# forgi86/pyMPC

Hardware: AMD Instinct MI355X
Metric: QP-solves/sec (MPC steps/sec) at nx=12 nu=4 Np=30; max |u*-u*_ref| (higher is better)
Workload: dtype f64

## Files before the change

include/mpcqp.h:

```cpp
#ifndef MPCQP_H
#define MPCQP_H

#include <stdint.h>

#ifdef __cplusplus
extern "C" {
#endif

typedef struct mpcqp_handle mpcqp_handle;

enum mpcqp_error {
    MPCQP_OK = 0,
    MPCQP_ERR_ARG = -1,
    MPCQP_ERR_HIP = -2,
    MPCQP_ERR_NO_DEVICE = -3,
    MPCQP_ERR_UNSUPPORTED = -4,
    MPCQP_ERR_STATE = -5
};

enum mpcqp_status {
    MPCQP_SOLVED = 1, MPCQP_SOLVED_INACCURATE = 2, MPCQP_MAX_ITER_REACHED = -2,
    MPCQP_PRIMAL_INFEASIBLE = -3, MPCQP_PRIMAL_INFEASIBLE_INACCURATE = 3,
    MPCQP_DUAL_INFEASIBLE = -4, MPCQP_DUAL_INFEASIBLE_INACCURATE = 4,
    MPCQP_NON_CVX = -7, MPCQP_UNSOLVED = -10
// ... 16 lines not shown
    MPCQP_BACKEND_SWEEPS = 1,
    MPCQP_BACKEND_DENSE = 2,
    MPCQP_BACKEND_BCR = 3,
    MPCQP_BACKEND_BCR8 = 4,
    MPCQP_BACKEND_BCRT = 5
};
enum mpcqp_tuning {
    MPCQP_TUNE_NO_BALANCE = 1,
    MPCQP_TUNE_NO_LSTAGE = 2,
    MPCQP_TUNE_NO_GROUPING = 4,
    MPCQP_TUNE_NO_W8 = 8,
    MPCQP_TUNE_NO_QUEUE = 16,
    MPCQP_TUNE_NO_PARTS = 32,
    MPCQP_TUNE_QUEUE_SOLVES = 64,
    MPCQP_TUNE_EVEN_PARTS = 128,
    MPCQP_TUNE_ONE_LAUNCH_SOLVES = 1 << 29,
    MPCQP_TUNE_NO_SHARE = 1 << 30,
    MPCQP_TUNE_SLOTS_SHIFT = 24,
    MPCQP_TUNE_PACE_SHIFT = 8
};

typedef struct {
    int32_t status;
    int32_t iter;
    int32_t rho_updates;
    int32_t reserved;
    double obj_val;
    double pri_res, dua_res;
    double rho;
} mpcqp_info;
// ... 109 lines not shown
```

pympc_amd/_lib.py:

```python
import ctypes as C
import os

_HERE = os.path.dirname(os.path.abspath(__file__))
LIB_PATH = os.path.join(_HERE, 'libmpcqp_hip.so')

SYMBOLS = [
    'mpcqp_default_settings', 'mpcqp_status_string', 'mpcqp_last_error', 'mpcqp_device_count',
    'mpcqp_create', 'mpcqp_destroy', 'mpcqp_set_stream', 'mpcqp_synchronize',
    'mpcqp_setup', 'mpcqp_setup_qp', 'mpcqp_create_csc', 'mpcqp_setup_csc', 'mpcqp_update', 'mpcqp_update_vectors', 'mpcqp_warm_start', 'mpcqp_update_settings', 'mpcqp_solve',
    'mpcqp_mpc_step', 'mpcqp_step_host', 'mpcqp_mpc_run', 'mpcqp_mpc_loop', 'mpcqp_get_solution', 'mpcqp_get_u0', 'mpcqp_get_shape', 'mpcqp_get_dims', 'mpcqp_get_stream_bytes', 'mpcqp_get_work', 'mpcqp_get_occupancy', 'mpcqp_kernel_name', 'mpcqp_get_stats', 'mpcqp_get_launch_times', 'mpcqp_profile',
    'mpcqp_export_qp', 'mpcqp_get_scaling', 'mpcqp_debug_kkt_solve', 'mpcqp_get_iterate', 'mpcqp_iterate', 'mpcqp_refactor', 'mpcqp_share_factor', 'mpcqp_eq_solve',
]


class Settings(C.Structure):
    _fields_ = [('rho', C.c_double), ('sigma', C.c_double), ('alpha', C.c_double),
                ('eps_abs', C.c_double), ('eps_rel', C.c_double),
                ('eps_prim_inf', C.c_double), ('eps_dual_inf', C.c_double),
                ('adaptive_rho_tolerance', C.c_double),
                ('max_iter', C.c_int32), ('check_termination', C.c_int32), ('scaling', C.c_int32),
                ('adaptive_rho', C.c_int32), ('adaptive_rho_interval', C.c_int32), ('warm_start', C.c_int32),
                ('soft_constraints', C.c_int32), ('backend', C.c_int32), ('tuning', C.c_int32)]


BACKEND_AUTO, BACKEND_SWEEPS, BACKEND_DENSE, BACKEND_BCR, BACKEND_BCR8, BACKEND_BCRT = 0, 1, 2, 3, 4, 5
TUNE_NO_BALANCE, TUNE_NO_LSTAGE, TUNE_NO_GROUPING, TUNE_NO_W8, TUNE_NO_QUEUE, TUNE_NO_PARTS = 1, 2, 4, 8, 16, 32
TUNE_NO_SHARE = 1 << 30
TUNE_PACE_SHIFT = 8


class Info(C.Structure):
    _fields_ = [('status', C.c_int32), ('iter', C.c_int32), ('rho_updates', C.c_int32), ('reserved', C.c_int32),
                ('obj_val', C.c_double), ('pri_res', C.c_double), ('dua_res', C.c_double), ('rho', C.c_double)]


_pd = C.POINTER(C.c_double)


class Model(C.Structure):
    _fields_ = [(k, _pd) for k in ('Ad', 'Bd', 'Qx', 'QxN', 'Qu', 'QDu', 'xmin', 'xmax', 'umin', 'umax',
                                   'Dumin', 'Dumax', 'uref', 'eps_feas')]

# ... 82 lines not shown
```

pympc_amd/csrc/mpcqp.hip:

```cpp

#include <hip/hip_runtime.h>
#include <math.h>
#include <stdint.h>
#include <stdio.h>
#include <string.h>
#include <sched.h>
#include <algorithm>
#include <cstdio>
#include <cstdlib>
#include <string>
#include <vector>

#include "../../include/mpcqp.h"

#include "mpcqp_defs.h"

static inline void cpu_relax() {
#if defined(__x86_64__) || defined(__i386__)
    __builtin_ia32_pause();
#elif defined(__aarch64__)
    __asm__ __volatile__("yield");
#else
    __asm__ __volatile__("" ::: "memory");
#endif
// ... 42 lines not shown
    int device, batch;
    Lay L;
    Ptrs P;
    mpcqp_settings S;
    hipStream_t stream;
    bool own_stream, is_setup, lds_state;
    size_t smem_setup, smem_solve;
    std::vector<void *> allocs;
    double *u0_dev;
    int *pending_dev, *npending_dev;
    int *perm_dev;
    int *qperm_dev; bool qperm_set;
    int *vcur_dev, *vdone_dev; unsigned *vqueue_dev;
    std::vector<double> work_ema;
    int ncu, solves_since_balance, auto_balance;
    void *run_buf; size_t run_bytes;
    bool profiling;
    hipEvent_t ev0[MAXEV], ev1[MAXEV];
    long long ev_count;
    double run_ms;
    long long run_launches;
    int nevents;
    bool warm_x_pending;
    double *pin_in, *pin_out; void *pin_in_dev, *pin_out_dev;
    unsigned *done_dev; unsigned long long host_seq; int pin_stride; bool pin_tried;
    PackArgs pack;
    CscSeam *csc;
    double *vec_buf;
    bool step_blank;
    int *fown_dev; unsigned *nshared_dev;
// ... 71 lines not shown
    HIPCHK(hipMalloc(&q, count * sizeof(T) + 16));
    HIPCHK(hipMemsetAsync(q, 0, count * sizeof(T) + 16, h->stream));
    h->allocs.push_back(q);
    *p = (T *)q;
    return 0;
}

extern "C" int mpcqp_create(mpcqp_handle **out, int device, int batch, int nx, int nu, int Np, int Nc, const mpcqp_settings *s) {
    if (!out || batch < 1 || nx < 1 || nu < 1 || Np < 2 || Nc < 1 || Nc > Np) return fail(MPCQP_ERR_ARG, "mpcqp_create: bad dimensions");
    if (nx + nu > 128) return fail(MPCQP_ERR_UNSUPPORTED, "mpcqp_create: nx+nu > 128 is not implemented");
    int ndev = 0;
    if (hipGetDeviceCount(&ndev) != hipSuccess || ndev == 0) return fail(MPCQP_ERR_NO_DEVICE, "no HIP device available");
    if (device < 0 || device >= ndev) return fail(MPCQP_ERR_ARG, "mpcqp_create: bad device index");
    HIPCHK(hipSetDevice(device));
    mpcqp_handle *h = new mpcqp_handle();
    h->device = device; h->batch = batch; h->is_setup = false; h->u0_dev = nullptr; h->run_buf = nullptr; h->run_bytes = 0; h->perm_dev = nullptr; h->vcur_dev = nullptr; h->vdone_dev = nullptr; h->vqueue_dev = nullptr; h->qperm_dev = nullptr; h->qperm_set = false; h->solves_since_balance = 0; h->auto_balance = 1; h->ncu = 0;
    h->profiling = false; h->run_ms = 0.0; h->run_launches = 0; h->ev_count = 0; h->nevents = 0; h->stream = nullptr; h->own_stream = false;
    h->warm_x_pending = false;
    h->csc = nullptr; h->vec_buf = nullptr; h->step_blank = false;
    h->pin_in = h->pin_out = nullptr; h->pin_in_dev = h->pin_out_dev = nullptr; h->done_dev = nullptr; h->host_seq = 0; h->pin_stride = 0; h->pin_tried = false;
    if (s) h->S = *s; else mpcqp_default_settings(&h->S);
    h->L = make_layout(nx, nu, Np, Nc, h->S.soft_constraints);
    auto hip_fail = [&](hipError_t e, const char *what) { std::string msg = std::string(what) + ": " + hipGetErrorString(e); mpcqp_destroy(h); return fail(MPCQP_ERR_HIP, msg); };
    { hipError_t e = hipStreamCreate(&h->stream); if (e != hipSuccess) { h->stream = nullptr; return hip_fail(e, "hipStreamCreate"); } }
    h->own_stream = true;
    for (int i = 0; i < MAXEV; ++i) {
        hipError_t e = hipEventCreate(&h->ev0[i]); if (e != hipSuccess) return hip_fail(e, "hipEventCreate");
        e = hipEventCreate(&h->ev1[i]); if (e != hipSuccess) { hipEventDestroy(h->ev0[i]); return hip_fail(e, "hipEventCreate"); }
        h->nevents = i + 1;
    }
    const Lay &L = h->L;
// ... 35 lines not shown
                  : (long long)L.fhead + (long long)L.N * L.fstage;
    int rc = 0;
    rc |= dalloc(h, &P.model, B * L.model_sz); rc |= dalloc(h, &P.step, B * L.step_sz);
    rc |= dalloc(h, &P.D, B * L.n); rc |= dalloc(h, &P.E, B * L.m); rc |= dalloc(h, &P.c, B);
    rc |= dalloc(h, &P.omega, B * L.m); rc |= dalloc(h, &P.s, B * L.n); rc |= dalloc(h, &P.rho, B);
    rc |= dalloc(h, &P.F, (B + 1) * (size_t)P.fsz);
    rc |= dalloc(h, &h->fown_dev, B); rc |= dalloc(h, &h->nshared_dev, 4);
    rc |= dalloc(h, &P.x, B * L.n); rc |= dalloc(h, &P.z, B * L.m); rc |= dalloc(h, &P.y, B * L.m);
    rc |= dalloc(h, &P.xo, B * L.n); rc |= dalloc(h, &P.yo, B * L.m);
    rc |= dalloc(h, &P.dx, B * L.n); rc |= dalloc(h, &P.dy, B * L.m);
    rc |= dalloc(h, &P.qv, B * (size_t)(L.n_x + L.n_u));
    if (bcr) rc |= dalloc(h, &P.bws, B * (size_t)NS * BcrFmt::WSTAGE);
    if (L.NB == 128) rc |= dalloc(h, &P.bws, B * (size_t)HugeFmt::GWS);
    if (L.border) { rc |= dalloc(h, &P.Bb, B * (size_t)L.nu * L.N * L.NB); rc |= dalloc(h, &P.Zb, B * (size_t)L.nu * L.N * L.NB); rc |= dalloc(h, &P.Sig, B * (size_t)L.nu * L.nu); }
    rc |= dalloc(h, &P.Dt, B * L.n); rc |= dalloc(h, &P.Et, B * L.m);
    rc |= dalloc(h, &P.ctype, B * L.m); rc |= dalloc(h, &P.info, B); rc |= dalloc(h, &P.stats, 8);
        rc |= dalloc(h, &h->u0_dev, B * L.nu);
    rc |= dalloc(h, &P.work, B); rc |= dalloc(h, &h->perm_dev, B);
    rc |= dalloc(h, &h->vcur_dev, (size_t)std::max(4 * h->ncu, 1)); rc |= dalloc(h, &h->vqueue_dev, 4); rc |= dalloc(h, &h->vdone_dev, B); rc |= dalloc(h, &h->qperm_dev, B);
    rc |= dalloc(h, &P.tstamp, (size_t)TS_STRIDE * B);
    rc |= dalloc(h, &h->pending_dev, B); rc |= dalloc(h, &h->npending_dev, 4);
    if (h->S.tuning & MPCQP_TUNE_NO_BALANCE) h->auto_balance = 0;
    if (rc) { std::string msg = g_err; mpcqp_destroy(h); return fail(MPCQP_ERR_HIP, msg); }
    const int toplds = bcrt ? LATW_TOP_LDS(NS) + 2 : 0;
    const int fws = dense ? L.NR * L.dld + 2 * DenseFmt::ROWS + L.m + L.n : bcr ? BcrFmt::lds_doubles(h->L.nw, L.m + L.n, bcrt ? BcrFmt::top_count(NS) : 0) : (L.NB == 16 ? FactorCfg<16>::WS : L.NB == 32 ? FactorCfg<32>::WS : L.NB == 64 ? WideFmt::WS : HugeFmt::WS);
    const int need = std::max(fws, (L.border && !dense) ? 2 * L.nu * L.nu : 0);
    const int avail = L.tsz + (h->lds_state ? (int)state_doubles : 0) + toplds;
    if (avail < need) h->L.tsz += need - avail;
    h->smem_setup = sizeof(double) * ((size_t)smem_common_doubles(h->L) + (h->lds_state ? state_doubles : 0) + (size_t)toplds);
    {
        const size_t stage_doubles = 2 * (size_t)L.n + 3 * (size_t)L.m + (size_t)(L.n_x + L.n_u) + (L.border ? 2 * (size_t)L.nu * L.N * L.NB + (size_t)L.nu * L.nu : 0);
// ... 307 lines not shown
    const int full = h->ncu * occ;
    const int q = (h->S.tuning >> MPCQP_TUNE_SLOTS_SHIFT) & 0x1F;
    if (q) return std::max(1, std::min(full, h->ncu * q / 8));
    if (L.NB == 32 && occ == 2 && !h->lds_state && !L.lstage && nsteps >= 8 && 2 * h->batch <= 3 * full && 4 * h->batch > 3 * full && !(h->S.tuning & MPCQP_TUNE_NO_QUEUE)) return 3 * full / 4;
    return full;
}
static RunKArgs run_kernel_args(mpcqp_handle *h, const RunArgs &R0, int *grid) {
    RunKArgs A; A.L = h->L; A.P = h->P; A.S = h->S; A.R = R0;
    *grid = h->batch;
    const int slots = run_grid(h, R0.nsteps);
    if (h->ncu > 0 && h->batch > slots && h->vcur_dev && !R0.pin_in && !R0.pub && (R0.nsteps > 0 || (h->S.tuning & (MPCQP_TUNE_QUEUE_SOLVES | MPCQP_TUNE_ONE_LAUNCH_SOLVES))) && !(h->S.tuning & MPCQP_TUNE_NO_QUEUE)) {
        A.R.vcur = h->vcur_dev; A.R.vperm = ((R0.nsteps > 0 || (R0.part == 0 && (h->S.tuning & MPCQP_TUNE_ONE_LAUNCH_SOLVES))) && h->qperm_set) ? h->qperm_dev : h->P.perm;       A.R.vqueue = h->vqueue_dev;
        A.P.perm = h->vcur_dev;
        *grid = slots;
        if (R0.nsteps > 1 && !(h->S.tuning & MPCQP_TUNE_NO_PARTS)) {
            const int per_slot = ((h->S.tuning >> 16) & 0xFF) ? ((h->S.tuning >> 16) & 0xFF) : QUEUE_ITEMS_PER_SLOT;
            const int parts = std::min(R0.nsteps, (per_slot * slots + h->batch - 1) / h->batch);
            if (parts > 1) {
                const int np = std::min(parts, 16);
                int off = 0;
                for (int p = 0; p < np; ++p) {
                    A.R.voff[p] = off;
                    const int left = R0.nsteps - off, pl = np - p;
                    int len = pl == 1 ? left : std::max(1, std::min(left - (pl - 1), (2 * left + pl) / (pl + 1)));
                    if (h->S.tuning & MPCQP_TUNE_EVEN_PARTS) len = pl == 1 ? left : (left + pl - 1) / pl;
                    off += len;
                }
                A.R.voff[np] = R0.nsteps; A.R.vparts = np; A.R.vdone = h->vdone_dev;
            }
        }
    }
    return A;
}
template <int NB, bool LDSS, int NXT, int NUT, int MODE>
static int launch_run_t(mpcqp_handle *h, const RunArgs &R) {
    int grid;
    const RunKArgs A = run_kernel_args(h, R, &grid);
    if (A.R.vdone && hipMemsetAsync(h->vdone_dev, 0, sizeof(int) * (size_t)h->batch, h->stream) != hipSuccess) return MPCQP_ERR_HIP;
    if (R.nsteps > 0) {
        if (set_smem(k_mpc_run<NB, LDSS, NXT, NUT, MODE, true>, h->smem_solve)) return MPCQP_ERR_HIP;
        hipLaunchKernelGGL((k_mpc_run<NB, LDSS, NXT, NUT, MODE, true>), dim3(grid), dim3(NT), h->smem_solve, h->stream, A);
    } else {
        if (set_smem(k_mpc_run<NB, LDSS, NXT, NUT, MODE, false>, h->smem_solve)) return MPCQP_ERR_HIP;
        hipLaunchKernelGGL((k_mpc_run<NB, LDSS, NXT, NUT, MODE, false>), dim3(grid), dim3(NT), h->smem_solve, h->stream, A);
    }
    return 0;
// ... 381 lines not shown
    for (unsigned long long spins = 0; *flag != h->host_seq; ++spins) {
        if (spins < 20000) cpu_relax(); else sched_yield();
        if ((spins & 0xfffff) == 0xfffff) {
            hipError_t e = hipStreamQuery(h->stream);
            if (e != hipSuccess && e != hipErrorNotReady) return fail(MPCQP_ERR_HIP, std::string("mpcqp_step_host: ") + hipGetErrorString(e));
            if (e == hipSuccess && *flag != h->host_seq) { HIPCHK(hipStreamSynchronize(h->stream)); break; }
        }
    }
    __atomic_thread_fence(__ATOMIC_ACQUIRE);
    if (x) memcpy(x, h->pin_out, sizeof(double) * B * L.n);
    if (y) memcpy(y, h->pin_out + B * L.n, sizeof(double) * B * L.m);
    if (info) memcpy(info, h->pin_out + B * (L.n + L.m), sizeof(mpcqp_info) * B);
    return MPCQP_OK;
}

extern "C" int mpcqp_get_stats(mpcqp_handle *h, uint64_t *out4, int reset) {
    if (!h || !out4) return fail(MPCQP_ERR_ARG, "null argument");
    HIPCHK(hipSetDevice(h->device));
    HIPCHK(hipMemcpyAsync(out4, h->P.stats, 4 * sizeof(uint64_t), hipMemcpyDefault, h->stream));
#ifdef MPCQP_RUN_TIMING
    { uint64_t t[4]; hipMemcpy(t, h->P.stats + 4, sizeof(t), hipMemcpyDeviceToHost); fprintf(stderr, "phase wall-clock ticks: begin %llu admm %llu check %llu\n", (unsigned long long)t[0], (unsigned long long)t[1], (unsigned long long)t[2]);
      unsigned long long g[16]; hipMemcpyFromSymbol(g, HIP_SYMBOL(g_ticks), sizeof(g)); unsigned long long z[16] = {0}; hipMemcpyToSymbol(HIP_SYMBOL(g_ticks), z, sizeof(z));
      if (h->L.nw == 8) mpcqp_w8_ticks(g);
      { double tot = 0; for (int i = 0; i < 7; ++i) tot += (double)g[i]; if (tot <= 0) tot = 1;
        fprintf(stderr, "iteration cycles (thread 0, summed over workgroups): rhs %.1f%% fwd %.1f%% middle %.1f%% bwd %.1f%% t4 %.1f%% t5 %.1f%% t6 %.1f%% total %.3g;  outside the iterations (same unit): t7 %.3g t8 %.3g t9 %.3g;  check: setup+tail %.3g rows %.3g vars %.3g reduce %.3g decide %.3g\n",
                100 * g[0] / tot, 100 * g[1] / tot, 100 * g[2] / tot, 100 * g[3] / tot, 100 * g[4] / tot, 100 * g[5] / tot, 100 * g[6] / tot, tot, (double)g[7], (double)g[8], (double)g[9], (double)g[10], (double)g[11], (double)g[12], (double)g[13], (double)g[14]); } }
#endif
    if (reset) HIPCHK(hipMemsetAsync(h->P.stats, 0, 8 * sizeof(uint64_t), h->stream));
    HIPCHK(hipStreamSynchronize(h->stream));
    return MPCQP_OK;
}

extern "C" int mpcqp_get_launch_times(mpcqp_handle *h, uint64_t *out, int nsteps) {
    if (!h || !out || nsteps < 0 || nsteps > TS_STEPS) return fail(MPCQP_ERR_ARG, "mpcqp_get_launch_times: bad argument (0 <= nsteps <= 64)");
    HIPCHK(hipSetDevice(h->device));
    HIPCHK(hipMemcpy2DAsync(out, sizeof(uint64_t) * (size_t)(2 + nsteps), h->P.tstamp, sizeof(uint64_t) * (size_t)TS_STRIDE, sizeof(uint64_t) * (size_t)(2 + nsteps),
                            (size_t)h->batch, hipMemcpyDefault, h->stream));
    HIPCHK(hipStreamSynchronize(h->stream));
    return MPCQP_OK;
}

extern "C" int mpcqp_profile(mpcqp_handle *h, int enable, double *run_ms, int64_t *run_launches, int reset) {
    if (!h) return fail(MPCQP_ERR_ARG, "null handle");
// ... 187 lines not shown
```

pympc_amd/csrc/mpcqp_kernels.h:

```cpp
#pragma once


struct RunSmem { Smem S; double *X, *Z, *Y; };
template <bool LDSSTATE>
__device__ __forceinline__ RunSmem run_smem(const Lay &L, const Ptrs &P) {
    extern __shared__ __attribute__((aligned(16))) double sh[];
    RunSmem r; double *p = sh; smem_common(L, P, p, r.S);
    r.X = r.Z = r.Y = nullptr;
    if (LDSSTATE) { r.X = carve(p, L.n); r.Z = carve(p, L.m); r.Y = carve(p, L.m); }
    return r;
}

template <int OCC>
__device__ __noinline__ void run_group_factor_phase(int *frame_pin) {
    PHASE_PIN_USE(frame_pin);
    const RunKArgs &A = run_kargs();
    const Lay &L = A.L; const Ptrs &P = A.P;
    RunSmem r = run_smem<false>(L, P);
    const int b = inst_of(P.perm);
    factor_unshare(P, b);
    Ctx c{L, r.S.hot, P.model + (size_t)b * L.model_sz + L.hot_sz};
    factor_grouped(c, P.omega + (size_t)b * L.m, P.s + (size_t)b * L.n, P.c[b], P.F + (size_t)b * P.fsz, r.S.T, r.S.iflag, border_ptrs(L, P, r.S));
}

// ... 59 lines not shown
__device__ __forceinline__ void run_instance(const int k0, const int k1) {
    constexpr int OCC = run_occupancy(NB, MODE);
    const RunKArgs &A = run_kargs();
    const Lay &L = A.L; const Ptrs &P = A.P; const RunArgs &R = A.R;
    RunSmem rs = run_smem<LDSSTATE>(L, P);
    Smem &S = rs.S;
    const int b = inst_of(P.perm), tid = threadIdx.x;
    double *step = P.step + (size_t)b * L.step_sz;
    if (LOOP && tid == 0 && k0 == 0) P.tstamp[(size_t)TS_STRIDE * b] = wall_clock64();
    if (LOOP && tid == 0 && k0 == 0 && R.nsteps < TS_STEPS) {
        unsigned hw, xcc;
        asm volatile("s_getreg_b32 %0, hwreg(HW_REG_HW_ID)" : "=s"(hw));
        asm volatile("s_getreg_b32 %0, hwreg(HW_REG_XCC_ID)" : "=s"(xcc));
        P.tstamp[(size_t)TS_STRIDE * b + 2 + TS_STEPS - 1] = ((unsigned long long)(xcc & 15) << 32) | hw;
    }
    if (MODE >= MODE_BCRT && tid == 0) S.iflag[2] = 0;
    const double *step_src = step;
    if (!LOOP && R.inl_n) {
        for (int i = tid; i < R.inl_n; i += NT) step[i] = R.inl[i];
        step_src = R.inl;
    } else if (!LOOP && R.pin_in) {
        const double *src = R.pin_in + (size_t)b * R.pin_stride;
        if (R.pin_mask & 1) for (int i = tid; i < L.nx; i += NT) step[i] = src[i];
        if (R.pin_mask & 2) for (int i = tid; i < L.nu; i += NT) step[L.nx + i] = src[L.nx + i];
        if (R.pin_mask & 4) for (int i = tid; i < R.pin_xref; i += NT) step[L.nx + L.nu + i] = src[L.nx + L.nu + i];
        __syncthreads();
    }
    load_common(L, P.model + (size_t)b * L.model_sz, step_src, S);
    if (!LOOP && R.part == 3) {
        __syncthreads();
        { FramePin pin; run_factor_phase<NB, OCC>(&pin.v); }
        return;
    }
    const int nx = L.nx, nu = L.nu;
    for (int k = k0; k < k1; ++k) {
        if (LOOP) {
            double *un = S.T, *xn = S.T + 128, *xt = S.T + 256, *ym = S.T + 384, *inn = S.T + 512, *xu = S.T + 640;
            const size_t kb = (size_t)k * R.batch + b;
            const int ny = R.ny;
            const int status = k > k0 ? S.iflag[4] : P.info[b].status;
            if (tid < nu) un[tid] = status == MPCQP_SOLVED ? (k > k0 ? S.uo[tid] : P.xo[(size_t)b * L.n + L.ou + tid]) : S.hot[L.ouref + tid];
            if (tid < nx) xt[tid] = ny ? R.x_true[(size_t)b * nx + tid] : S.x0s[tid];
            __syncthreads();
            if (ny && tid < ny) {
                const double *C = R.C + (size_t)b * ny * nx + (size_t)tid * nx;
                double y = R.v ? R.v[kb * ny + tid] : 0.0, yh = 0.0;
                for (int j = 0; j < nx; ++j) { y += C[j] * xt[j]; yh += C[j] * S.x0s[j]; }
                ym[tid] = y; inn[tid] = y - yh;
                if (R.y_traj) R.y_traj[kb * ny + tid] = y;
            }
            if (tid < nx) {
// ... 19 lines not shown
                __syncthreads();
                if (tid < nx) {
                    const double *Ad = S.hot + L.oAd, *Bd = S.hot + L.oBd;
                    double acc = 0.0;
                    for (int j = 0; j < nx; ++j) acc += Ad[tid * nx + j] * xu[j];
                    for (int j = 0; j < nu; ++j) acc += Bd[tid * nu + j] * un[j];
                    xn[tid] = acc;
                }
                __syncthreads();
            }
            if (tid < nx) { S.x0s[tid] = xn[tid]; step[tid] = xn[tid]; }
            if (tid < nu) { S.um1s[tid] = un[tid]; step[nx + tid] = un[tid]; S.du0[tid] = S.hot[L.oDumin + tid] + un[tid]; S.du0[nu + tid] = S.hot[L.oDumax + tid] + un[tid]; }
            if (R.xref_traj) for (int i = tid; i < R.xref_blk; i += NT) { const double xr = R.xref_traj[kb * R.xref_blk + i]; step[nx + nu + i] = xr; if (i < nx) S.xrs[i] = xr; }
            __syncthreads();
        }
#ifdef MPCQP_RUN_TIMING
#define PHASE_CLOCK(i) { unsigned long long t_ = wall_clock64(); if (tid == 0) atomicAdd(&P.stats[4 + (i)], t_ - tphase); tphase = t_; }
        unsigned long long tphase = wall_clock64();
#else
#define PHASE_CLOCK(i)
#endif
        int iter = 0, term = 0;
        if (!LOOP && R.part == 2) {
            const mpcqp_info pi = P.info[b];
            iter = pi.iter;
            if (tid == 0) { S.iflag[1] = pi.rho_updates; S.iflag[3] = pi.reserved; }
        }
        else { FramePin pin; run_begin_phase<NB, LDSSTATE, OCC>(R.plain, (R.warm_x && k == 0) ? 1 : 0, &pin.v); }
        __syncthreads();
        PHASE_CLOCK(0)
        while (!term) {
            const int nxt = next_stop(iter, R.max_iter, R.chk, R.rho_every);
            term = __builtin_amdgcn_readfirstlane(run_admm<NB, LDSSTATE, NXT, NUT, MODE, OCC>(nxt - iter, R.plain ? -1 : iter));
            iter = nxt;
            __syncthreads();
            if constexpr (MODE >= MODE_BCRT) { if (!R.plain) iter = S.iflag[5]; }
            PHASE_CLOCK(1)
            if (term) break;
            { FramePin pin; term = run_check_phase<NB, LDSSTATE, OCC>(iter, stop_mode(iter, R.max_iter, R.chk, R.rho_every, R.plain != 0), &pin.v); }
            __syncthreads();
            PHASE_CLOCK(2)
            if (!LOOP && R.part == 1 && !term) {
                if (tid == 0) R.pending[atomicAdd(R.npending, 1)] = b;
                break;
            }
        }
        if (LOOP && tid == 0) {
            R.status_traj[(size_t)k * R.batch + b] = S.iflag[4];
            R.iter_traj[(size_t)k * R.batch + b] = iter;
            if (k < TS_STEPS) P.tstamp[(size_t)TS_STRIDE * b + 2 + k] = wall_clock64();
        }
        __syncthreads();
    }
    if (!LOOP && R.pub) {
        double *px = R.pub + (size_t)b * L.n, *py = R.pub + (size_t)R.batch * L.n + (size_t)b * L.m;
        for (int j = tid; j < L.n; j += NT) px[j] = P.xo[(size_t)b * L.n + j];
        for (int r = tid; r < L.m; r += NT) py[r] = P.yo[(size_t)b * L.m + r];
        mpcqp_info *pi = (mpcqp_info *)(R.pub + (size_t)R.batch * (L.n + L.m));
        if (tid == 0) pi[b] = P.info[b];
        __threadfence_system();
// ... 28 lines not shown
    const int nvirt = (!LOOP && R.part == 2) ? *R.npending : R.batch;
    const int nparts = (LOOP && R.vparts > 1) ? R.vparts : 1;
    for (;;) {
        if (threadIdx.x == 0) {
            const int v = (int)atomicAdd(R.vqueue, 1u);
            int entry = -1, ka = 0, kb = nrun;
            if (v < nvirt * nparts) {
                const int part = v / nvirt, idx = v - part * nvirt;
                entry = R.vperm ? R.vperm[idx] : idx;
                if (nparts > 1) { ka = R.voff[part]; kb = R.voff[part + 1]; }
                if (part > 0) {
                    volatile int *done = R.vdone + (entry & PERM_INST_MASK);
                    while (*done < ka) __builtin_amdgcn_s_sleep(16);
                }
                R.vcur[blockIdx.x] = entry;
            }
            s_item[0] = entry; s_item[1] = ka; s_item[2] = kb;
        }
        __syncthreads();
        const int entry = s_item[0], ka = s_item[1], kb = s_item[2];
        if (entry < 0) {
            if (threadIdx.x == 0 && atomicAdd(R.vqueue + 1, 1u) == gridDim.x - 1) { R.vqueue[1] = 0; __threadfence(); R.vqueue[0] = 0; }
            break;
        }
        __builtin_amdgcn_s_dcache_inv();
        __builtin_amdgcn_fence(__ATOMIC_ACQUIRE, "agent");
        run_instance<NB, LDSSTATE, NXT, NUT, MODE, LOOP>(ka, kb);
        __syncthreads();
        if (nparts > 1 && threadIdx.x == 0) { __threadfence(); *(volatile int *)(R.vdone + (entry & PERM_INST_MASK)) = kb; }
    }
}

template <int NB>
__global__ __launch_bounds__(NT) void k_export(Lay L, Ptrs P, double *Pd, double *Ad_, double *q, double *l, double *u) {
    extern __shared__ __attribute__((aligned(16))) double sh[];
    double *p = sh; Smem S; smem_common(L, P, p, S);
    const int b = inst_of(P.perm), tid = threadIdx.x;
    const double *model = P.model + (size_t)b * L.model_sz, *step = P.step + (size_t)b * L.step_sz;
    load_common(L, model, step, S);
    Ctx c{L, S.hot, model + L.hot_sz};
    if (!L.raw) build_q(c, step, S.Qv);
    __syncthreads();
// ... 132 lines not shown
```

pympc_amd/csrc/mpcqp_latw.h:

```cpp
#pragma once

constexpr int latw_owner(int , int , int kind, int t) { return kind == 1 ? NWAVES - 1 - t % NWAVES : t % NWAVES; }
#ifndef LATW_FUSE0
#define LATW_FUSE0 2
#endif
constexpr bool latw_fused(int N) { return LATW_FUSE0 && (N + 3) / 4 == NWAVES; }
constexpr bool latw_fused_back(int N) { return LATW_FUSE0 >= 2 && latw_fused(N); }
constexpr int LATW_F0 = 6;
constexpr int LATW_FB = 6;
constexpr int latw_slot(int N, int W, int Lq, int kq, int tq) {
    int s = latw_fused(N) ? LATW_F0 : 0;
    for (int pass = 0; pass < 2; ++pass)
        for (int li = 0; li < 2; ++li) {
            const int L = pass == 0 ? li : 1 - li;
            for (int kind = (pass == 0 ? 0 : 2); kind < (pass == 0 ? 2 : 3); ++kind)
                for (int t = 0; t < lat_count(N, L, kind); ++t) {
                    if (latw_fused(N) && L == 0 && kind < 2) continue;
                    if (latw_fused_back(N) && kind == 2) continue;
                    if (L == Lq && kind == kq && t == tq) return s;
                    if (latw_owner(N, L, kind, t) == W) s += lat_nfr(N, L, kind, t);
                }
        }
    return s;
}
// ... 308 lines not shown
    if constexpr (latw_fused_back(N)) {
        LATW_DISPATCH(wv, (latw_bwd_own<N, W>(fr, v)))
        TICK(4)
    } else {
        LATW_DISPATCH(wv, (latw_bwd1<N, W>(fr, v)))
        __syncthreads();
        TICK(4)
        LATW_DISPATCH(wv, (latw_bwd<N, W, 0, false>(fr, v)))
    }
}

enum { LATW_CONTINUE = 0, LATW_SOLVED = 1, LATW_GENERIC = 2 };
template <int NXT, int NUT, int NST>
__device__ int latw_check(double pv, double pv2, double ncq, double zA, double ysA, double omA, double zB, double ysB, double omB, double z0, double ys0, double om0,
                          double loA, double hiA, double loB, double hiB, double cc, int iter, int *frame_pin);

template <int NXT, int NUT, int NST>
__device__ __forceinline__ int admm_latw(const Lay &L, const HotPtrs &P, Smem &S, double *Xl, double *Zl, double *Yl, double alpha, int iters, int iter0) {
    constexpr int NB = 16, N = NST, NG = (N + 3) / 4, QN = (NG + NWAVES - 1) / NWAVES;
#ifdef MPCQP_RUN_TIMING
    const unsigned long long tf0_ = clock64();
#endif
#ifndef LATW_FAST
#define LATW_FAST 1
#endif
    const bool fast = LATW_FAST && iter0 >= 0 && L.hot_lds > L.hot_sz;
    static_assert(NXT + NUT <= NB, "16 x 16 stages");
    const int nx = NXT ? NXT : L.nx, nu = NUT ? NUT : L.nu, NR = L.N;
    const int b = inst_of(P.perm), tid = threadIdx.x, lane = tid & 63, wv = __builtin_amdgcn_readfirstlane(tid >> 6);
    gdouble *gx = (gdouble *)(P.x + (size_t)b * L.n), *gz = (gdouble *)(P.z + (size_t)b * L.m), *gy = (gdouble *)(P.y + (size_t)b * L.m);
// ... 151 lines not shown
        }
        __syncthreads();
        TICK(6)
    }
    iter += iters;
    if (!fast) break;
    TICK_START
    if constexpr (QN != 1) break;
    else {
        const RunArgs &R = run_kargs().R;
        if (stop_mode(iter, R.max_iter, R.chk, R.rho_every, R.plain != 0) != COLD_CHECK) break;
        int verdict;
        { FramePin pin; verdict = latw_check<NXT, NUT, NST>(pv[0], pv2[0], ncq[0], rA[0].z, rA[0].ys, rA[0].om, rB[0].z, rB[0].ys, rB[0].om, r0.z, r0.ys, r0.om,
                                                               loA[0], hiA[0], loB[0], hiB[0], cc, iter, &pin.v); }
        verdict = __builtin_amdgcn_readfirstlane(verdict);
        if (verdict == LATW_SOLVED) { term = 1; break; }
        if (verdict != LATW_CONTINUE) break;
        iters = next_stop(iter, R.max_iter, R.chk, R.rho_every) - iter;
        auto rt = [&](LatRow &r) { r.ys = cc * (r.ys * (r.om * cinv)) / r.om; r.w = r.om * (r.z - r.ys); };
        rt(rA[0]); rt(rB[0]);
        if (u0v) rt(r0);
        WA[sl[0]] = ok[0] ? rA[0].w : 0.0; WB[sl[0]] = ok[0] ? rB[0].w : 0.0;
        __syncthreads();
    }
    TICK(9)
    }
    TICK_START
    if (!term) {
        auto put_row = [&](const LatRow &r, int idx) { const double y = r.ys * (r.om * cinv); gz[idx] = r.z; gy[idx] = y; Zl[idx] = r.z; Yl[idx] = y; };
#pragma unroll
        for (int q = 0; q < QN; ++q) {
            if (ok[q]) {
// ... 16 lines not shown
```

pympc_amd/csrc/mpcqp_latw_check.h:

```cpp
#pragma once

template <int NXT, int NUT, int NST>
__device__ __noinline__ int latw_check(double pv, double pv2, double ncq, double zA, double ysA, double omA, double zB, double ysB, double omB, double z0, double ys0, double om0,
                                       double loA, double hiA, double loB, double hiB, double cc, int iter, int *frame_pin) {
    PHASE_PIN_USE(frame_pin);
    constexpr int NB = 16, N = NST, NG = (N + 3) / 4, VS = LAT_VS(N), NTOP = BcrFmt::top_count(N);
    static_assert(NG <= NWAVES, "one group of four stages per wave");
    const RunKArgs &KA = run_kargs();
    const Lay &L = KA.L; const Ptrs &PP = KA.P; const RunArgs &R = KA.R;
    RunSmem rs = run_smem<true>(L, PP);
    Smem &S = rs.S;
    const int nx = NXT ? NXT : L.nx, nu = NUT ? NUT : L.nu, NR = L.N;
    const int b = inst_of(PP.perm), tid = threadIdx.x, lane = tid & 63, wv = __builtin_amdgcn_readfirstlane(tid >> 6);
    const double cinv = 1.0 / cc;
    const double *hot = S.hot;
    double *Tc = S.T + NB, *Cc = Tc + VS;
    const double *TopL = rs.Y + L.m + ((smem_common_doubles(L) + L.n + 2 * L.m) & 1);
    const int a = 4 * ((lane >> 2) & 3) + (lane >> 4), J = lane & 3;
    const bool is_x = a < nx;
    const int jj = a - nx;
    const int s = wv < NG ? 4 * wv + J : 4 * NG, sl = s * NB + a;
    const bool ok = is_x ? s < NR : (a < nx + nu && s < NR - 1);
    const int e = s * nx + a, cu = s * nu + jj;
    const int pidx = is_x ? e : L.ou + cu, aidx = is_x ? e : L.ri + cu, bidx = is_x ? L.rs + e : L.rdu + nu + cu;
// ... 83 lines not shown
            S.iflag[4] = MPCQP_SOLVED;
            atomicAdd(&PP.stats[0], (unsigned long long)iter); atomicAdd(&PP.stats[1], (unsigned long long)inf.reserved);
            atomicAdd(&PP.stats[2], (unsigned long long)inf.rho_updates); atomicAdd(&PP.stats[3], 1ULL);
            PP.work[b] += (unsigned)iter;
            inf.reserved = 0;
            PP.info[b] = inf;
        }
        return LATW_SOLVED;
    }
    if (R.nsteps == 0 && R.part == 1) return LATW_GENERIC;
    if (!pc && nrm[7] > epi && vsum[1] < -epi * nrm[7]) return LATW_GENERIC;
    if (!dc && nrm[8] > edi && vsum[2] < -edi * nrm[8]) return LATW_GENERIC;
    if (tid == 0) S.iflag[3] += 1;
    return LATW_CONTINUE;
}
```

pympc_amd/csrc/mpcqp_qp.h:

```cpp
#pragma once

__device__ __forceinline__ double input_weight(double iu, double qu, double dk, double qdu) {
    double a = iu * qu, b = dk * qdu;
    asm volatile("" : "+v"(a), "+v"(b));
    return a + b;
}


template <class F>
__device__ __forceinline__ void A_row(const Ctx &c, int r, F f) {
    const Lay &L = c.L;
    if (r < L.rs) {
        int k = idiv(r, L.rnx), i = r - k * L.nx;
        f(-1.0, r);
        if (k > 0) {
            const double *a = c.Ad() + i * L.nx;
            int base = (k - 1) * L.nx;
            for (int j = 0; j < L.nx; ++j) f(a[j], base + j);
            int ku = min(k - 1, L.Nc - 1);
            const double *b = c.Bd() + i * L.nu;
            base = L.ou + ku * L.nu;
            for (int j = 0; j < L.nu; ++j) f(b[j], base + j);
        }
    } else if (r < L.ri) {
// ... 76 lines not shown
    } else if (r < L.ri) {
        int j = r - L.rs; int k = idiv(j, L.rnx); int i = j - k * L.nx;
        lo = c.hot[L.oxmin + i]; hi = c.hot[L.oxmax + i];
    } else if (r < L.rdu) {
        int cc = r - L.ri; int k = idiv(cc, L.rnu); int jj = cc - k * L.nu;
        lo = c.hot[L.oumin + jj]; hi = c.hot[L.oumax + jj];
    } else {
        int rr = r - L.rdu; int k = idiv(rr, L.rnu); int jj = rr - k * L.nu;
        lo = c.hot[L.oDumin + jj]; hi = c.hot[L.oDumax + jj];
        if (rr < L.nu) { lo = du0[jj]; hi = du0[L.nu + jj]; }
    }
    lo = lo < -QP_INFTY ? -QP_INFTY : lo;
    hi = hi > QP_INFTY ? QP_INFTY : hi;
}

__device__ __forceinline__ void build_q(const Ctx &c, const double *step, double *Qv, const double *um1s = nullptr, const double *xrs = nullptr) {
    const Lay &L = c.L;
    const double *um1 = um1s ? um1s : step + L.nx, *xref = xrs ? xrs : step + L.nx + L.nu;
    const double *uref = c.hot + L.ouref;
    for (int j = threadIdx.x; j < L.n_x + L.n_u; j += NT) {
        double acc = 0.0;
        if (j < L.n_x) {
            int k = idiv(j, L.rnx), i = j - k * L.nx;
            const double *Q = (k < L.Np) ? c.Qx() : c.QxN();
            if (L.xref_rows == 1) { for (int l = 0; l < L.nx; ++l) acc += Q[i * L.nx + l] * xref[l]; }
            else { const double *xr = xref + k * L.nx; for (int l = 0; l < L.nx; ++l) acc += xr[l] * Q[l * L.nx + i]; }
            acc = -acc;
        } else {
            int cc = j - L.n_x; int k = idiv(cc, L.rnu), jj = cc - k * L.nu;
            double iu = (k == L.Nc - 1) ? (double)(L.Np - L.Nc + 1) : 1.0;
            double a = 0.0;
            for (int l = 0; l < L.nu; ++l) a += c.Qu()[jj * L.nu + l] * uref[l];
            acc = iu * (-a);
            if (k == 0) { double d = 0.0; for (int l = 0; l < L.nu; ++l) d += c.QDu()[jj * L.nu + l] * um1[l]; acc += -d; }
        }
        Qv[j] = acc;
    }
    __syncthreads();
}

template <int CTRL>
__device__ __forceinline__ double dpp_move_f64(double x) {
    const long long xi = __builtin_bit_cast(long long, x);
    const int lo = __builtin_amdgcn_mov_dpp((int)xi, CTRL, 0xF, 0xF, false), hi = __builtin_amdgcn_mov_dpp((int)(xi >> 32), CTRL, 0xF, 0xF, false);
    return __builtin_bit_cast(double, ((long long)hi << 32) | (unsigned)lo);
}
__device__ __forceinline__ double readlane_f64(double x, int l) {
    const long long xi = __builtin_bit_cast(long long, x);
    const int lo = __builtin_amdgcn_readlane((int)xi, l), hi = __builtin_amdgcn_readlane((int)(xi >> 32), l);
// ... 118 lines not shown
```

pympc_amd/solver.py:

```python
import ctypes as C
import math

import numpy as np

from . import _lib

_SETTING_NAMES = [f[0] for f in _lib.Settings._fields_]
_IGNORED_SETTINGS = ('verbose', 'polish', 'linsys_solver', 'time_limit', 'scaled_termination', 'delta',
                     'polish_refine_iter', 'adaptive_rho_fraction')


_FIXED_AT_CREATE = ('rho', 'sigma', 'scaling', 'soft_constraints', 'backend', 'tuning')

_STATUS_STRINGS = {}


def _ptr(a):
    if a is None:
        return None
    if hasattr(a, 'data_ptr'):
        return C.c_void_p(a.data_ptr())
    return C.c_void_p(a.ctypes.data)


# ... 346 lines not shown
        info = (_lib.Info * self.batch)()
        _lib.check(self._L.mpcqp_get_solution(self._h, None, None, C.cast(info, C.c_void_p)), 'mpcqp_get_solution')
        return info

    def u0(self, out=None):
        if out is None:
            out = np.empty((self.batch, self.nu))
        _lib.check(self._L.mpcqp_get_u0(self._h, _ptr(out)), 'mpcqp_get_u0')
        return out

    def stats(self, reset=False):
        out = (C.c_uint64 * 4)()
        _lib.check(self._L.mpcqp_get_stats(self._h, out, int(bool(reset))), 'mpcqp_get_stats')
        return tuple(int(v) for v in out)

    def stream_bytes(self):
        a, b, c = C.c_int64(), C.c_int64(), C.c_int64()
        _lib.check(self._L.mpcqp_get_stream_bytes(self._h, C.byref(a), C.byref(b), C.byref(c)), 'mpcqp_get_stream_bytes')
        return a.value, b.value, c.value

    def mfma_per_iter(self):
        v = C.c_int64()
        _lib.check(self._L.mpcqp_get_work(self._h, C.byref(v)), 'mpcqp_get_work')
        return v.value

    def occupancy(self):
        a, b, c = C.c_int(), C.c_int(), C.c_int()
        _lib.check(self._L.mpcqp_get_occupancy(self._h, C.byref(a), C.byref(b), C.byref(c)), 'mpcqp_get_occupancy')
        return a.value, b.value, c.value

# ... 158 lines not shown
```

Before: 1.997 million.

## Carry closed-loop MPC steps inside the ADMM loop without leaving the solver

In the fused closed-loop run kernel, when a step's QP is solved, the new latw_carry path simulates the plant, updates x0/u-1, the q vector and the bounds in place, and keeps iterating on the next step without exiting and re-entering the solver. If the active constraint-type pattern changes, it falls back to the normal per-step path. The goal is to remove the per-step setup and exit overhead between consecutive MPC steps. In exchange it adds branch complexity, extra fences and a new tuning flag to disable it, plus stats counters.

```diff
diff --git a/include/mpcqp.h b/include/mpcqp.h
--- a/include/mpcqp.h
+++ b/include/mpcqp.h
@@ -54,6 +54,8 @@
     MPCQP_TUNE_NO_PARTS = 32,
     MPCQP_TUNE_QUEUE_SOLVES = 64,
     MPCQP_TUNE_EVEN_PARTS = 128,
+    MPCQP_TUNE_ITEMS_SHIFT = 16,
+    MPCQP_TUNE_NO_CARRY = 1 << 23,
     MPCQP_TUNE_ONE_LAUNCH_SOLVES = 1 << 29,
     MPCQP_TUNE_NO_SHARE = 1 << 30,
     MPCQP_TUNE_SLOTS_SHIFT = 24,
diff --git a/pympc_amd/_lib.py b/pympc_amd/_lib.py
--- a/pympc_amd/_lib.py
+++ b/pympc_amd/_lib.py
@@ -26,6 +26,8 @@
 BACKEND_AUTO, BACKEND_SWEEPS, BACKEND_DENSE, BACKEND_BCR, BACKEND_BCR8, BACKEND_BCRT = 0, 1, 2, 3, 4, 5
 TUNE_NO_BALANCE, TUNE_NO_LSTAGE, TUNE_NO_GROUPING, TUNE_NO_W8, TUNE_NO_QUEUE, TUNE_NO_PARTS = 1, 2, 4, 8, 16, 32
 TUNE_NO_SHARE = 1 << 30
+TUNE_ITEMS_SHIFT = 16
+TUNE_NO_CARRY = 1 << 23
 TUNE_PACE_SHIFT = 8
 
 
diff --git a/pympc_amd/csrc/mpcqp.hip b/pympc_amd/csrc/mpcqp.hip
--- a/pympc_amd/csrc/mpcqp.hip
+++ b/pympc_amd/csrc/mpcqp.hip
@@ -80,6 +80,7 @@
     int *vcur_dev, *vdone_dev; unsigned *vqueue_dev;
     std::vector<double> work_ema;
     int ncu, solves_since_balance, auto_balance;
+    int loop_parts;
     void *run_buf; size_t run_bytes;
     bool profiling;
     hipEvent_t ev0[MAXEV], ev1[MAXEV];
@@ -181,7 +182,7 @@
     if (device < 0 || device >= ndev) return fail(MPCQP_ERR_ARG, "mpcqp_create: bad device index");
     HIPCHK(hipSetDevice(device));
     mpcqp_handle *h = new mpcqp_handle();
-    h->device = device; h->batch = batch; h->is_setup = false; h->u0_dev = nullptr; h->run_buf = nullptr; h->run_bytes = 0; h->perm_dev = nullptr; h->vcur_dev = nullptr; h->vdone_dev = nullptr; h->vqueue_dev = nullptr; h->qperm_dev = nullptr; h->qperm_set = false; h->solves_since_balance = 0; h->auto_balance = 1; h->ncu = 0;
+    h->device = device; h->batch = batch; h->is_setup = false; h->u0_dev = nullptr; h->run_buf = nullptr; h->run_bytes = 0; h->perm_dev = nullptr; h->vcur_dev = nullptr; h->vdone_dev = nullptr; h->vqueue_dev = nullptr; h->qperm_dev = nullptr; h->qperm_set = false; h->solves_since_balance = 0; h->auto_balance = 1; h->ncu = 0; h->loop_parts = 0;
     h->profiling = false; h->run_ms = 0.0; h->run_launches = 0; h->ev_count = 0; h->nevents = 0; h->stream = nullptr; h->own_stream = false;
     h->warm_x_pending = false;
     h->csc = nullptr; h->vec_buf = nullptr; h->step_blank = false;
@@ -247,7 +248,7 @@
     if (L.NB == 128) rc |= dalloc(h, &P.bws, B * (size_t)HugeFmt::GWS);
     if (L.border) { rc |= dalloc(h, &P.Bb, B * (size_t)L.nu * L.N * L.NB); rc |= dalloc(h, &P.Zb, B * (size_t)L.nu * L.N * L.NB); rc |= dalloc(h, &P.Sig, B * (size_t)L.nu * L.nu); }
     rc |= dalloc(h, &P.Dt, B * L.n); rc |= dalloc(h, &P.Et, B * L.m);
-    rc |= dalloc(h, &P.ctype, B * L.m); rc |= dalloc(h, &P.info, B); rc |= dalloc(h, &P.stats, 8);
+    rc |= dalloc(h, &P.ctype, B * L.m); rc |= dalloc(h, &P.info, B); rc |= dalloc(h, &P.stats, 10);
         rc |= dalloc(h, &h->u0_dev, B * L.nu);
     rc |= dalloc(h, &P.work, B); rc |= dalloc(h, &h->perm_dev, B);
     rc |= dalloc(h, &h->vcur_dev, (size_t)std::max(4 * h->ncu, 1)); rc |= dalloc(h, &h->vqueue_dev, 4); rc |= dalloc(h, &h->vdone_dev, B); rc |= dalloc(h, &h->qperm_dev, B);
@@ -585,7 +586,8 @@
         A.P.perm = h->vcur_dev;
         *grid = slots;
         if (R0.nsteps > 1 && !(h->S.tuning & MPCQP_TUNE_NO_PARTS)) {
-            const int per_slot = ((h->S.tuning >> 16) & 0xFF) ? ((h->S.tuning >> 16) & 0xFF) : QUEUE_ITEMS_PER_SLOT;
+            const int ov = (h->S.tuning >> MPCQP_TUNE_ITEMS_SHIFT) & 0x7F;
+            const int per_slot = ov ? ov : QUEUE_ITEMS_PER_SLOT;
             const int parts = std::min(R0.nsteps, (per_slot * slots + h->batch - 1) / h->batch);
             if (parts > 1) {
                 const int np = std::min(parts, 16);
@@ -601,6 +603,7 @@
             }
         }
     }
+    if (R0.nsteps > 0) h->loop_parts = A.R.vcur ? std::max(1, A.R.vparts) : 0;
     return A;
 }
 template <int NB, bool LDSS, int NXT, int NUT, int MODE>
@@ -1012,19 +1015,28 @@
     return MPCQP_OK;
 }
 
+extern "C" int mpcqp_dev_carry_stats(mpcqp_handle *h, uint64_t *out3) {
+    if (!h || !out3) return fail(MPCQP_ERR_ARG, "null argument");
+    HIPCHK(hipSetDevice(h->device));
+    HIPCHK(hipMemcpyAsync(out3, h->P.stats + 8, 2 * sizeof(uint64_t), hipMemcpyDefault, h->stream));
+    HIPCHK(hipStreamSynchronize(h->stream));
+    out3[2] = (uint64_t)h->loop_parts;
+    return MPCQP_OK;
+}
+
 extern "C" int mpcqp_get_stats(mpcqp_handle *h, uint64_t *out4, int reset) {
     if (!h || !out4) return fail(MPCQP_ERR_ARG, "null argument");
     HIPCHK(hipSetDevice(h->device));
     HIPCHK(hipMemcpyAsync(out4, h->P.stats, 4 * sizeof(uint64_t), hipMemcpyDefault, h->stream));
 #ifdef MPCQP_RUN_TIMING
-    { uint64_t t[4]; hipMemcpy(t, h->P.stats + 4, sizeof(t), hipMemcpyDeviceToHost); fprintf(stderr, "phase wall-clock ticks: begin %llu admm %llu check %llu\n", (unsigned long long)t[0], (unsigned long long)t[1], (unsigned long long)t[2]);
+    { uint64_t t[4]; hipMemcpy(t, h->P.stats + 4, sizeof(t), hipMemcpyDeviceToHost); fprintf(stderr, "phase wall-clock ticks: begin %llu admm %llu check %llu body %llu\n", (unsigned long long)t[0], (unsigned long long)t[1], (unsigned long long)t[2], (unsigned long long)t[3]);
       unsigned long long g[16]; hipMemcpyFromSymbol(g, HIP_SYMBOL(g_ticks), sizeof(g)); unsigned long long z[16] = {0}; hipMemcpyToSymbol(HIP_SYMBOL(g_ticks), z, sizeof(z));
       if (h->L.nw == 8) mpcqp_w8_ticks(g);
       { double tot = 0; for (int i = 0; i < 7; ++i) tot += (double)g[i]; if (tot <= 0) tot = 1;
         fprintf(stderr, "iteration cycles (thread 0, summed over workgroups): rhs %.1f%% fwd %.1f%% middle %.1f%% bwd %.1f%% t4 %.1f%% t5 %.1f%% t6 %.1f%% total %.3g;  outside the iterations (same unit): t7 %.3g t8 %.3g t9 %.3g;  check: setup+tail %.3g rows %.3g vars %.3g reduce %.3g decide %.3g\n",
                 100 * g[0] / tot, 100 * g[1] / tot, 100 * g[2] / tot, 100 * g[3] / tot, 100 * g[4] / tot, 100 * g[5] / tot, 100 * g[6] / tot, tot, (double)g[7], (double)g[8], (double)g[9], (double)g[10], (double)g[11], (double)g[12], (double)g[13], (double)g[14]); } }
 #endif
-    if (reset) HIPCHK(hipMemsetAsync(h->P.stats, 0, 8 * sizeof(uint64_t), h->stream));
+    if (reset) HIPCHK(hipMemsetAsync(h->P.stats, 0, 10 * sizeof(uint64_t), h->stream));
     HIPCHK(hipStreamSynchronize(h->stream));
     return MPCQP_OK;
 }
diff --git a/pympc_amd/csrc/mpcqp_kernels.h b/pympc_amd/csrc/mpcqp_kernels.h
--- a/pympc_amd/csrc/mpcqp_kernels.h
+++ b/pympc_amd/csrc/mpcqp_kernels.h
@@ -97,7 +97,7 @@
         asm volatile("s_getreg_b32 %0, hwreg(HW_REG_XCC_ID)" : "=s"(xcc));
         P.tstamp[(size_t)TS_STRIDE * b + 2 + TS_STEPS - 1] = ((unsigned long long)(xcc & 15) << 32) | hw;
     }
-    if (MODE >= MODE_BCRT && tid == 0) S.iflag[2] = 0;
+    if (MODE >= MODE_BCRT && tid == 0) { S.iflag[2] = 0; S.iflag[6] = 0; S.iflag[7] = 0; }
     const double *step_src = step;
     if (!LOOP && R.inl_n) {
         for (int i = tid; i < R.inl_n; i += NT) step[i] = R.inl[i];
@@ -116,8 +116,13 @@
         return;
     }
     const int nx = L.nx, nu = L.nu;
+    const bool carry = LOOP && MODE >= MODE_BCRT && !(A.S.tuning & MPCQP_TUNE_NO_CARRY) && R.ny == 0 && !R.xref_traj && !R.plain && A.S.warm_start && !L.raw;
+    bool stepped = false;
     for (int k = k0; k < k1; ++k) {
-        if (LOOP) {
+#ifdef MPCQP_RUN_TIMING
+        const unsigned long long tbody = wall_clock64();
+#endif
+        if (LOOP && !stepped) {
             double *un = S.T, *xn = S.T + 128, *xt = S.T + 256, *ym = S.T + 384, *inn = S.T + 512, *xu = S.T + 640;
             const size_t kb = (size_t)k * R.batch + b;
             const int ny = R.ny;
@@ -167,9 +172,12 @@
             if (R.xref_traj) for (int i = tid; i < R.xref_blk; i += NT) { const double xr = R.xref_traj[kb * R.xref_blk + i]; step[nx + nu + i] = xr; if (i < nx) S.xrs[i] = xr; }
             __syncthreads();
         }
+        stepped = false;
+        if (carry && tid == 0) { S.iflag[6] = k; S.iflag[7] = k1; }
 #ifdef MPCQP_RUN_TIMING
 #define PHASE_CLOCK(i) { unsigned long long t_ = wall_clock64(); if (tid == 0) atomicAdd(&P.stats[4 + (i)], t_ - tphase); tphase = t_; }
         unsigned long long tphase = wall_clock64();
+        if (LOOP && tid == 0) atomicAdd(&P.stats[7], tphase - tbody);
 #else
 #define PHASE_CLOCK(i)
 #endif
@@ -197,6 +205,10 @@
                 if (tid == 0) R.pending[atomicAdd(R.npending, 1)] = b;
                 break;
             }
+        }
+        if (carry) {
+            k = __builtin_amdgcn_readfirstlane(S.iflag[6]);
+            if (__builtin_amdgcn_readfirstlane(S.iflag[7]) < 0) { stepped = true; --k; __syncthreads(); continue; }
         }
         if (LOOP && tid == 0) {
             R.status_traj[(size_t)k * R.batch + b] = S.iflag[4];
@@ -255,6 +267,7 @@
                     while (*done < ka) __builtin_amdgcn_s_sleep(16);
                 }
                 R.vcur[blockIdx.x] = entry;
+                __threadfence();
             }
             s_item[0] = entry; s_item[1] = ka; s_item[2] = kb;
         }
@@ -267,6 +280,7 @@
         __builtin_amdgcn_s_dcache_inv();
         __builtin_amdgcn_fence(__ATOMIC_ACQUIRE, "agent");
         run_instance<NB, LDSSTATE, NXT, NUT, MODE, LOOP>(ka, kb);
+        if (nparts > 1) __threadfence();
         __syncthreads();
         if (nparts > 1 && threadIdx.x == 0) { __threadfence(); *(volatile int *)(R.vdone + (entry & PERM_INST_MASK)) = kb; }
     }
diff --git a/pympc_amd/csrc/mpcqp_latw.h b/pympc_amd/csrc/mpcqp_latw.h
--- a/pympc_amd/csrc/mpcqp_latw.h
+++ b/pympc_amd/csrc/mpcqp_latw.h
@@ -346,6 +346,8 @@
 template <int NXT, int NUT, int NST>
 __device__ int latw_check(double pv, double pv2, double ncq, double zA, double ysA, double omA, double zB, double ysB, double omB, double z0, double ys0, double om0,
                           double loA, double hiA, double loB, double hiB, double cc, int iter, int *frame_pin);
+template <int NXT, int NUT, int NST>
+__device__ int latw_carry(int iter, int *frame_pin);
 
 template <int NXT, int NUT, int NST>
 __device__ __forceinline__ int admm_latw(const Lay &L, const HotPtrs &P, Smem &S, double *Xl, double *Zl, double *Yl, double alpha, int iters, int iter0) {
@@ -527,8 +529,16 @@
         { FramePin pin; verdict = latw_check<NXT, NUT, NST>(pv[0], pv2[0], ncq[0], rA[0].z, rA[0].ys, rA[0].om, rB[0].z, rB[0].ys, rB[0].om, r0.z, r0.ys, r0.om,
                                                                loA[0], hiA[0], loB[0], hiB[0], cc, iter, &pin.v); }
         verdict = __builtin_amdgcn_readfirstlane(verdict);
-        if (verdict == LATW_SOLVED) { term = 1; break; }
-        if (verdict != LATW_CONTINUE) break;
+        if (verdict == LATW_SOLVED) {
+            const int kc = __builtin_amdgcn_readfirstlane(S.iflag[6]), ke = __builtin_amdgcn_readfirstlane(S.iflag[7]);
+            if (!(R.nsteps > 0 && kc >= 0 && ke <= R.nsteps && kc + 1 < ke)) { term = 1; break; }
+            int carried;
+            { FramePin pin; carried = latw_carry<NXT, NUT, NST>(iter, &pin.v); }
+            if (!__builtin_amdgcn_readfirstlane(carried)) { term = 1; break; }
+            if (u0v) ncq[0] = Tc[sl[0]];
+            if (is_x && wv == 0 && (lane & 3) == 0) { loA[0] = Cc[sl[0]]; hiA[0] = loA[0]; }
+            iter = 0;
+        } else if (verdict != LATW_CONTINUE) break;
         iters = next_stop(iter, R.max_iter, R.chk, R.rho_every) - iter;
         auto rt = [&](LatRow &r) { r.ys = cc * (r.ys * (r.om * cinv)) / r.om; r.w = r.om * (r.z - r.ys); };
         rt(rA[0]); rt(rB[0]);
diff --git a/pympc_amd/csrc/mpcqp_latw_check.h b/pympc_amd/csrc/mpcqp_latw_check.h
--- a/pympc_amd/csrc/mpcqp_latw_check.h
+++ b/pympc_amd/csrc/mpcqp_latw_check.h
@@ -121,3 +121,70 @@
     if (tid == 0) S.iflag[3] += 1;
     return LATW_CONTINUE;
 }
+
+template <int NXT, int NUT, int NST>
+__device__ __noinline__ int latw_carry(int iter, int *frame_pin) {
+    PHASE_PIN_USE(frame_pin);
+#ifdef MPCQP_RUN_TIMING
+    const unsigned long long tw0_ = wall_clock64();
+#endif
+    constexpr int NB = 16, VS = LAT_VS(NST);
+    const RunKArgs &KA = run_kargs();
+    const Lay &L = KA.L; const Ptrs &P = KA.P; const RunArgs &R = KA.R;
+    RunSmem rs = run_smem<true>(L, P);
+    Smem &S = rs.S;
+    const int nx = NXT ? NXT : L.nx, nu = NUT ? NUT : L.nu;
+    const int b = inst_of(P.perm), tid = threadIdx.x;
+    double *step = P.step + (size_t)b * L.step_sz;
+    const int k = S.iflag[6], k1 = k + 1;
+    const size_t kb = (size_t)k1 * R.batch + b;
+    const int r = tid < nx ? tid : (tid < nx + nu ? L.rdu + (tid - nx) : -1);
+    const double v = (tid < nx && R.w) ? R.w[kb * nx + tid] : 0.0;
+    const double Er = r >= 0 ? P.E[(size_t)b * L.m + r] : 0.0;
+    const int ct = r >= 0 ? P.ctype[(size_t)b * L.m + r] : 0;
+    const double rho = P.rho[b], cc = P.c[b];
+    __syncthreads();
+    if (tid == 0) {
+        R.status_traj[(size_t)k * R.batch + b] = S.iflag[4];
+        R.iter_traj[(size_t)k * R.batch + b] = iter;
+        if (k < TS_STEPS) P.tstamp[(size_t)TS_STRIDE * b + 2 + k] = wall_clock64();
+    }
+    const double *un = S.uo, *xt = S.x0s;
+    double xn = 0.0;
+    if (tid < nx) {
+        const double *Ap = R.Ap ? R.Ap + (size_t)b * nx * nx : S.hot + L.oAd;
+        const double *Bp = R.Bp ? R.Bp + (size_t)b * nx * nu : S.hot + L.oBd;
+        double acc = 0.0;
+        for (int j = 0; j < nx; ++j) acc += Ap[tid * nx + j] * xt[j];
+        for (int j = 0; j < nu; ++j) acc += Bp[tid * nu + j] * un[j];
+        xn = acc + v;
+        R.x_traj[kb * nx + tid] = xt[tid];
+    }
+    if (tid < nu) R.u_traj[kb * nu + tid] = un[tid];
+    __syncthreads();
+    if (tid < nx) { S.x0s[tid] = xn; step[tid] = xn; }
+    if (tid < nu) { const double u = un[tid]; S.um1s[tid] = u; step[nx + tid] = u; S.du0[tid] = S.hot[L.oDumin + tid] + u; S.du0[nu + tid] = S.hot[L.oDumax + tid] + u; }
+    __syncthreads();
+    const Ctx c{L, S.hot, S.hot + L.hot_sz};
+    double *Tc = S.T + NB, *Cc = Tc + VS;
+    if (tid < nu) { const double qj = q_input(c, 0, tid, S.um1s, S.hot + L.ouref); S.Qv[L.n_x + tid] = qj; Tc[nx + tid] = -cc * qj; }
+    if (tid < nx) Cc[tid] = -S.x0s[tid];
+    int changed = 0;
+    if (r >= 0) { double lo, hi; row_bounds(c, S.x0s, S.du0, r, lo, hi); changed = row_type(Er, lo, hi) != ct; }
+    changed = __syncthreads_or(changed);
+    if (tid == 0) {
+        S.iflag[6] = k1;
+        atomicAdd(&P.stats[8], 1ULL);
+        if (changed) { S.iflag[7] = -1; atomicAdd(&P.stats[9], 1ULL); }
+        else {
+            mpcqp_info *inf = P.info + b;
+            inf->status = MPCQP_UNSOLVED; inf->iter = 0; inf->rho_updates = 0; inf->reserved = 0;
+            inf->obj_val = 0.0; inf->pri_res = 0.0; inf->dua_res = 0.0; inf->rho = rho;
+            S.iflag[1] = 0; S.iflag[3] = 0;
+        }
+    }
+#ifdef MPCQP_RUN_TIMING
+    if (tid == 0) atomicAdd(&P.stats[7], wall_clock64() - tw0_);
+#endif
+    return changed ? 0 : 1;
+}
diff --git a/pympc_amd/csrc/mpcqp_qp.h b/pympc_amd/csrc/mpcqp_qp.h
--- a/pympc_amd/csrc/mpcqp_qp.h
+++ b/pympc_amd/csrc/mpcqp_qp.h
@@ -114,6 +114,16 @@
     hi = hi > QP_INFTY ? QP_INFTY : hi;
 }
 
+__device__ __forceinline__ double q_input(const Ctx &c, int k, int jj, const double *um1, const double *uref) {
+    const Lay &L = c.L;
+    double iu = (k == L.Nc - 1) ? (double)(L.Np - L.Nc + 1) : 1.0;
+    double a = 0.0;
+    for (int l = 0; l < L.nu; ++l) a += c.Qu()[jj * L.nu + l] * uref[l];
+    double acc = iu * (-a);
+    if (k == 0) { double d = 0.0; for (int l = 0; l < L.nu; ++l) d += c.QDu()[jj * L.nu + l] * um1[l]; acc += -d; }
+    return acc;
+}
+
 __device__ __forceinline__ void build_q(const Ctx &c, const double *step, double *Qv, const double *um1s = nullptr, const double *xrs = nullptr) {
     const Lay &L = c.L;
     const double *um1 = um1s ? um1s : step + L.nx, *xref = xrs ? xrs : step + L.nx + L.nu;
@@ -128,11 +138,7 @@
             acc = -acc;
         } else {
             int cc = j - L.n_x; int k = idiv(cc, L.rnu), jj = cc - k * L.nu;
-            double iu = (k == L.Nc - 1) ? (double)(L.Np - L.Nc + 1) : 1.0;
-            double a = 0.0;
-            for (int l = 0; l < L.nu; ++l) a += c.Qu()[jj * L.nu + l] * uref[l];
-            acc = iu * (-a);
-            if (k == 0) { double d = 0.0; for (int l = 0; l < L.nu; ++l) d += c.QDu()[jj * L.nu + l] * um1[l]; acc += -d; }
+            acc = q_input(c, k, jj, um1, uref);
         }
         Qv[j] = acc;
     }
diff --git a/pympc_amd/solver.py b/pympc_amd/solver.py
--- a/pympc_amd/solver.py
+++ b/pympc_amd/solver.py
@@ -384,6 +384,13 @@
         _lib.check(self._L.mpcqp_get_stats(self._h, out, int(bool(reset))), 'mpcqp_get_stats')
         return tuple(int(v) for v in out)
 
+    def carry_stats(self):
+        fn = self._L.mpcqp_dev_carry_stats
+        fn.argtypes = [C.c_void_p, C.POINTER(C.c_uint64)]
+        out = (C.c_uint64 * 3)()
+        _lib.check(fn(self._h, out), 'mpcqp_dev_carry_stats')
+        return tuple(int(v) for v in out)
+
     def stream_bytes(self):
         a, b, c = C.c_int64(), C.c_int64(), C.c_int64()
         _lib.check(self._L.mpcqp_get_stream_bytes(self._h, C.byref(a), C.byref(b), C.byref(c)), 'mpcqp_get_stream_bytes')
```

Measured after the change: 2.129 million, median of 6. 1.07x the previous value.
